# AiRyunn/BoT

Measured on NVIDIA B200. Metric: GAT layer fwd+bwd edges/sec (ogbn-proteins shape), higher is better.
Workload: dtype f32

## Files before the change

bot_b200/_lib.py:

```python
from __future__ import annotations

import ctypes as C
import os

_HERE = os.path.dirname(os.path.abspath(__file__))
LIB_PATH = os.environ.get("BOTGAT_LIB") or os.path.join(_HERE, "libbotgat.so")
ABI_VERSION = 5

c_i64p = C.POINTER(C.c_int64)
c_vp = C.c_void_p

ARRAYS = ("in_indptr", "in_indices", "in_eid", "out_indptr", "out_indices", "out_eid", "in_deg", "out_deg")
ORDER_IN, ORDER_OUT = 0, 1


class GraphInfo(C.Structure):
    _fields_ = [
        ("n_src", C.c_int64), ("n_dst", C.c_int64), ("n_edges", C.c_int64),
        ("max_in_deg", C.c_int64), ("max_out_deg", C.c_int64),
        ("has_zero_in_degree", C.c_int32), ("device", C.c_int32),
        ("n_slots_in", C.c_int64), ("n_slots_out", C.c_int64),
        ("in_eid_identity", C.c_int32), ("tiles_src", C.c_int32), ("tiles_dst", C.c_int32),
        ("n_seg_in", C.c_int32), ("n_seg_out", C.c_int32), ("reserved_", C.c_int32),
    ]


class EdgeSubset(C.Structure):
    _fields_ = [("indptr", c_vp), ("indices", c_vp), ("eid", c_vp), ("kept", c_vp), ("base", c_vp), ("seg_beg", c_vp), ("seg_end", c_vp)]


class FwdArgs(C.Structure):
    _fields_ = [
        ("H", C.c_int32), ("D", C.c_int32),
        ("ld_ft", C.c_int64), ("ld_out", C.c_int64),
        ("ft", c_vp), ("el", c_vp), ("er", c_vp), ("eb", c_vp),
        ("Hb", C.c_int32), ("col_parts", C.c_int32),
        ("am", c_vp), ("ee", c_vp), ("keep", c_vp), ("attn_mul", c_vp), ("src_scale", c_vp), ("dst_scale", c_vp),
        ("slope", C.c_float), ("attn_p", C.c_float), ("seed", C.c_uint64),
        ("out", c_vp), ("row_max", c_vp), ("row_sum", c_vp), ("scratch", c_vp),
        ("h_begin", C.c_int32), ("h_count", C.c_int32),
        ("res", c_vp), ("ld_res", C.c_int64), ("res2", c_vp), ("ld_res2", C.c_int64),
        ("ep_scale", c_vp), ("ep_shift", c_vp), ("y", c_vp), ("ld_y", C.c_int64),
        ("ep_relu", C.c_int32), ("reserved_", C.c_int32),
        ("subset", C.POINTER(EdgeSubset)),
    ]


class BwdArgs(C.Structure):
    _fields_ = [
        ("H", C.c_int32), ("D", C.c_int32),
        ("ld_ft", C.c_int64), ("ld_out", C.c_int64), ("ld_gft", C.c_int64),
        ("ft", c_vp), ("el", c_vp), ("er", c_vp), ("eb_out", c_vp),
        ("Hb", C.c_int32), ("phases", C.c_int32),
        ("am_out", c_vp), ("ee", c_vp), ("keep", c_vp), ("attn_mul", c_vp), ("src_scale", c_vp), ("dst_scale", c_vp),
        ("slope", C.c_float), ("attn_p", C.c_float), ("seed", C.c_uint64),
        ("out", c_vp), ("row_max", c_vp), ("row_sum", c_vp), ("gout", c_vp),
        ("drec", c_vp), ("gprime", c_vp), ("scratch", c_vp), ("gz", c_vp),
        ("grad_ft", c_vp), ("grad_el", c_vp), ("grad_ee", c_vp), ("ld_gee", C.c_int64), ("grad_er", c_vp),
        ("h_begin", C.c_int32), ("h_count", C.c_int32),
        ("subset_out", C.POINTER(EdgeSubset)),
    ]


SIGNATURES = {
    "botgat_abi_version": (C.c_int, []),
# ... 76 lines not shown
```

bot_b200/csrc/common.cuh:

```cuda
#pragma once

#include <atomic>
#include <cuda_runtime.h>
#include <stdint.h>
#include <stdio.h>

#include <type_traits>

#include "botgat.h"

namespace botgat {

void set_error(const char* fmt, ...);
const char* env_str(const char* name);
int64_t env_int(const char* name, int64_t dflt);
extern std::atomic<long long> g_launches;
#define BG_LAUNCHED(n) (::botgat::g_launches.fetch_add(n, std::memory_order_relaxed))

#define BG_CHECK(expr)                                                                  \
  do {                                                                                  \
    cudaError_t _e = (expr);                                                            \
    if (_e != cudaSuccess) {                                                            \
      ::botgat::set_error("%s:%d: %s -> %s", __FILE__, __LINE__, #expr, cudaGetErrorString(_e)); \
      return -2;                                                                        \
    }                                                                                   \
  } while (0)

#define BG_REQUIRE(cond, ...)            \
  do {                                   \
    if (!(cond)) {                       \
      ::botgat::set_error(__VA_ARGS__);  \
      return -1;                         \
    }                                    \
  } while (0)

struct DeviceGuard {
  int prev = -1;
  explicit DeviceGuard(int dev) {
    cudaGetDevice(&prev);
    if (dev != prev) cudaSetDevice(dev);
  }
  ~DeviceGuard() {
    int cur;
    cudaGetDevice(&cur);
    if (cur != prev && prev >= 0) cudaSetDevice(prev);
  }
};

template <typename K>
static inline int resident_grid(K kernel, int block_threads, int64_t blocks_of_work) {
  int dev = 0, sms = 148, per_sm = 1;
  cudaGetDevice(&dev);
  cudaDeviceGetAttribute(&sms, cudaDevAttrMultiProcessorCount, dev);
  if (cudaOccupancyMaxActiveBlocksPerMultiprocessor(&per_sm, kernel, block_threads, 0) != cudaSuccess || per_sm < 1) per_sm = 1;
  const int64_t resident = (int64_t)sms * per_sm;
  return (int)(blocks_of_work < 1 ? 1 : (blocks_of_work < resident ? blocks_of_work : resident));
}

}

struct botgat_graph {
  int device = 0;
  int sm_count = 148;
  int64_t n_src = 0, n_dst = 0, n_edges = 0;
  int64_t max_in_deg = 0, max_out_deg = 0;
  int has_zero_in_degree = 0;
  int32_t *in_indptr = nullptr, *in_indices = nullptr, *in_eid = nullptr;
  int32_t *out_indptr = nullptr, *out_indices = nullptr, *out_eid = nullptr;
  int32_t *in_deg = nullptr, *out_deg = nullptr;
  int in_eid_identity = 0;
  int32_t* out_tile_order = nullptr;
  int tiles_s = 1, tiles_d = 1;
  struct SegTable {
    int n_items = 0;
    int n_slots = 0;
    int n_split = 0;
    int32_t *row = nullptr, *beg = nullptr, *end = nullptr, *slot = nullptr;
    int32_t *split_rows = nullptr, *split_first = nullptr;
  } seg_in, seg_out;
};

namespace botgat {

#ifndef BG_WPB
#define BG_WPB 4
#endif
constexpr int kWarpsPerBlock = BG_WPB;
constexpr unsigned kFull = 0xffffffffu;

__device__ __forceinline__ float leaky_relu(float z, float slope) {
  return z > 0.f ? z : (z == -INFINITY ? -INFINITY : z * slope);
}

__device__ __forceinline__ float warp_max(float v) {
#pragma unroll
  for (int o = 16; o > 0; o >>= 1) v = fmaxf(v, __shfl_xor_sync(kFull, v, o));
  return v;
}
__device__ __forceinline__ float warp_sum(float v) {
#pragma unroll
  for (int o = 16; o > 0; o >>= 1) v += __shfl_xor_sync(kFull, v, o);
  return v;
}

__device__ __forceinline__ uint32_t philox_u32(uint64_t seed, uint32_t eid, uint32_t head) {
  uint32_t c0 = eid, c1 = head >> 2, c2 = 0x9E3779B9u, c3 = 0xBB67AE85u;
  uint32_t k0 = (uint32_t)seed, k1 = (uint32_t)(seed >> 32);
#pragma unroll
  for (int r = 0; r < 10; ++r) {
    uint32_t hi0 = __umulhi(0xD2511F53u, c0), lo0 = 0xD2511F53u * c0;
    uint32_t hi1 = __umulhi(0xCD9E8D57u, c2), lo1 = 0xCD9E8D57u * c2;
    uint32_t n0 = hi1 ^ c1 ^ k0, n1 = lo1, n2 = hi0 ^ c3 ^ k1, n3 = lo0;
    c0 = n0; c1 = n1; c2 = n2; c3 = n3;
    k0 += 0x9E3779B9u; k1 += 0xBB67AE85u;
  }
  uint32_t sel = head & 3u;
  return sel == 0 ? c0 : sel == 1 ? c1 : sel == 2 ? c2 : c3;
}
__device__ __forceinline__ float philox_dropout_mul(uint64_t seed, uint32_t eid, uint32_t head, float p, float inv_keep) {
  float u = (float)(philox_u32(seed, eid, head) >> 8) * (1.0f / 16777216.0f);
  return u >= p ? inv_keep : 0.f;
}

template <int VW> struct Vec;
// ... 119 lines not shown
```

bot_b200/csrc/edge_ops.cu:

```cuda
#include <cub/cub.cuh>
#include <thrust/iterator/counting_iterator.h>
#include <thrust/iterator/transform_iterator.h>

#include "common.cuh"

namespace botgat {

static int env_pf() {
  return (int)env_int("BOTGAT_PF", 0);
}

template <int PF> __device__ __forceinline__ float4 ld_rec4(const float* p) {
  float4 r;
  if constexpr (PF == 64)
    asm("ld.global.nc.L2::64B.v4.f32 {%0,%1,%2,%3}, [%4];" : "=f"(r.x), "=f"(r.y), "=f"(r.z), "=f"(r.w) : "l"(p));
  else if constexpr (PF == 128)
    asm("ld.global.nc.L2::128B.v4.f32 {%0,%1,%2,%3}, [%4];" : "=f"(r.x), "=f"(r.y), "=f"(r.z), "=f"(r.w) : "l"(p));
  else if constexpr (PF == 256)
    asm("ld.global.nc.L2::256B.v4.f32 {%0,%1,%2,%3}, [%4];" : "=f"(r.x), "=f"(r.y), "=f"(r.z), "=f"(r.w) : "l"(p));
  else
    r = __ldg(reinterpret_cast<const float4*>(p));
  return r;
}
template <int PF> __device__ __forceinline__ float2 ld_rec2(const float* p) {
// ... 9 lines not shown
  if constexpr (PF == 64) asm("ld.global.nc.L2::64B.f32 %0, [%1];" : "=f"(r) : "l"(p));
  else if constexpr (PF == 128) asm("ld.global.nc.L2::128B.f32 %0, [%1];" : "=f"(r) : "l"(p));
  else if constexpr (PF == 256) asm("ld.global.nc.L2::256B.f32 %0, [%1];" : "=f"(r) : "l"(p));
  else r = __ldg(p);
  return r;
}

constexpr int kHMax = 8;

template <int VEC, int PF> __device__ __forceinline__ void load_record(const float* rec, int H, float (&v)[kHMax]) {
  if constexpr (VEC == 4) {
#pragma unroll
    for (int q = 0; q < kHMax / 4; ++q) {
      if (q * 4 < H) {
        const float4 t = ld_rec4<PF>(rec + q * 4);
        v[q * 4] = t.x; v[q * 4 + 1] = t.y; v[q * 4 + 2] = t.z; v[q * 4 + 3] = t.w;
      }
    }
  } else if constexpr (VEC == 2) {
#pragma unroll
    for (int q = 0; q < kHMax / 2; ++q) {
      if (q * 2 < H) {
        const float2 t = ld_rec2<PF>(rec + q * 2);
        v[q * 2] = t.x; v[q * 2 + 1] = t.y;
      }
    }
  } else {
#pragma unroll
    for (int q = 0; q < kHMax; ++q)
      if (q < H) v[q] = ld_rec1<PF>(rec + q);
  }
}
template <int VEC> __device__ __forceinline__ void store_record(float* rec, int H, const float (&v)[kHMax]) {
  if constexpr (VEC == 4) {
#pragma unroll
    for (int q = 0; q < kHMax / 4; ++q)
      if (q * 4 < H) *reinterpret_cast<float4*>(rec + q * 4) = make_float4(v[q * 4], v[q * 4 + 1], v[q * 4 + 2], v[q * 4 + 3]);
  } else if constexpr (VEC == 2) {
#pragma unroll
    for (int q = 0; q < kHMax / 2; ++q)
      if (q * 2 < H) *reinterpret_cast<float2*>(rec + q * 2) = make_float2(v[q * 2], v[q * 2 + 1]);
  } else {
#pragma unroll
    for (int q = 0; q < kHMax; ++q)
      if (q < H) rec[q] = v[q];
  }
}

static int record_vec(const void* p, int64_t ld, int H) {
  auto fits = [&](int w) { return ld % w == 0 && ((uintptr_t)p % (4 * w)) == 0 && ((H + w - 1) / w) * w <= ld; };
  return fits(4) ? 4 : (fits(2) ? 2 : 1);
}

__global__ void k_pack_keep(int64_t n_edges, const uint8_t* __restrict__ keep, uint32_t* __restrict__ bits) {
  const int64_t n_round = (n_edges + 31) & ~(int64_t)31;
  for (int64_t e = blockIdx.x * (int64_t)blockDim.x + threadIdx.x; e < n_round; e += (int64_t)gridDim.x * blockDim.x) {
    const unsigned b = __ballot_sync(0xffffffffu, e < n_edges && __ldg(keep + e) != 0);
    if ((threadIdx.x & 31) == 0) bits[e >> 5] = b;
  }
}

struct KeptMap {
  const uint32_t* bits;
  const int32_t* base;
  __device__ __forceinline__ int64_t rank(int64_t x) const {
    return __ldg(base + (x >> 5)) + __popc(__ldg(bits + (x >> 5)) & ((1u << (x & 31)) - 1u));
  }
  __device__ __forceinline__ bool kept(int64_t p) const { return (__ldg(bits + (p >> 5)) >> (p & 31)) & 1u; }
};

template <int VEC, int PF>
__global__ void k_edge_stage(int64_t n_edges, int h0, int Hn, const int32_t* __restrict__ eid,
                             const int32_t* __restrict__ order,
                             const float* __restrict__ src, int64_t ld, const uint8_t* __restrict__ keep,
                             const uint32_t* __restrict__ keep_bits, float* __restrict__ dst,
                             const KeptMap km, const int32_t* __restrict__ indices,
                             int32_t* __restrict__ sub_indices, int32_t* __restrict__ sub_eid) {
  for (int64_t t = blockIdx.x * (int64_t)blockDim.x + threadIdx.x; t < n_edges; t += (int64_t)gridDim.x * blockDim.x) {
    const int64_t p = order ? __ldg(order + t) : t;
    int64_t q = p;
    if (km.bits) {
      if (!km.kept(p)) continue;
      q = km.rank(p);
    }
    const int64_t e = __ldg(eid + p);
    float v[kHMax];
#pragma unroll
    for (int c = 0; c < kHMax; ++c) v[c] = 0.f;
    if (src) load_record<VEC, PF>(src + e * ld + h0, Hn, v);
    const bool dropped = keep_bits ? !((__ldg(keep_bits + (e >> 5)) >> (e & 31)) & 1u) : (keep && !__ldg(keep + e));
#pragma unroll
    for (int c = 0; c < kHMax; ++c)
      if (c < Hn) dst[(int64_t)(h0 + c) * n_edges + q] = dropped ? -INFINITY : v[c];
    if (sub_indices) {
      sub_indices[q] = __ldg(indices + p);
      if (sub_eid) sub_eid[q] = (int32_t)e;
    }
  }
}

template <int VEC>
__global__ void k_edge_unstage(int64_t n_edges, int h0, int Hn, int Hw, const int32_t* __restrict__ eid,
                               const int32_t* __restrict__ order, const KeptMap km,
                               const float* __restrict__ gz, float* __restrict__ dst, int64_t ld) {
  for (int64_t t = blockIdx.x * (int64_t)blockDim.x + threadIdx.x; t < n_edges; t += (int64_t)gridDim.x * blockDim.x) {
    const int64_t p = order ? __ldg(order + t) : t;
    const int64_t e = __ldg(eid + p);
    int64_t q = p;
    bool kept = true;
    if (km.bits) {
      kept = km.kept(p);
      q = km.rank(p);
    }
    float v[kHMax];
#pragma unroll
    for (int c = 0; c < kHMax; ++c) v[c] = (c < Hn && kept) ? __ldg(gz + (int64_t)(h0 + c) * n_edges + q) : 0.f;
    store_record<VEC>(dst + e * ld + h0, Hw, v);
  }
}

__global__ void k_kept_bits(int64_t n_edges, int64_t n_words, const int32_t* __restrict__ eid, const uint8_t* __restrict__ keep,
                            const uint32_t* __restrict__ keep_bits, uint32_t* __restrict__ bits) {
  for (int64_t p = blockIdx.x * (int64_t)blockDim.x + threadIdx.x; p < n_words * 32; p += (int64_t)gridDim.x * blockDim.x) {
    bool k = false;
    if (p < n_edges) {
      const int64_t e = eid ? __ldg(eid + p) : p;
      k = keep_bits ? ((__ldg(keep_bits + (e >> 5)) >> (e & 31)) & 1u) : __ldg(keep + e) != 0;
    }
    const unsigned b = __ballot_sync(0xffffffffu, k);
    if ((threadIdx.x & 31) == 0) bits[p >> 5] = b;
  }
}

struct WordCount {
  const uint32_t* bits;
  __device__ int operator()(int64_t w) const { return __popc(__ldg(bits + w)); }
};

__global__ void k_subset_bounds(int n_rows, const int32_t* __restrict__ indptr, int n_seg, const int32_t* __restrict__ seg_beg,
                                const int32_t* __restrict__ seg_end, const KeptMap km,
                                int32_t* __restrict__ sub_indptr, int32_t* __restrict__ sub_beg, int32_t* __restrict__ sub_end) {
  const int n = max(n_rows + 1, n_seg);
  for (int i = blockIdx.x * blockDim.x + threadIdx.x; i < n; i += gridDim.x * blockDim.x) {
    if (i <= n_rows) sub_indptr[i] = (int32_t)km.rank(__ldg(indptr + i));
    if (i < n_seg) {
      sub_beg[i] = (int32_t)km.rank(__ldg(seg_beg + i));
      sub_end[i] = (int32_t)km.rank(__ldg(seg_end + i));
    }
  }
}

template <int VEC, int PF>
__global__ void __launch_bounds__(256)
k_edge_reduce_dst(int n_items, int H, int h0, int Hn, const int32_t* __restrict__ indptr, const int32_t* __restrict__ eid,
                  const int32_t* __restrict__ seg_row, const int32_t* __restrict__ seg_beg,
                  const int32_t* __restrict__ seg_end, const int32_t* __restrict__ seg_slot,
                  const float* __restrict__ grad_ee, int64_t ld, float* __restrict__ grad_er, float* __restrict__ scratch) {
  const int warp = threadIdx.x >> 5, lane = threadIdx.x & 31;
  const int item = blockIdx.x * 8 + warp;
  if (item >= n_items) return;
  const int v = seg_row ? seg_row[item] : item;
  const int beg = seg_row ? seg_beg[item] : indptr[v], end = seg_row ? seg_end[item] : indptr[v + 1];
  const int slot = seg_row ? seg_slot[item] : -1;
  float s[kHMax];
#pragma unroll
  for (int q = 0; q < kHMax; ++q) s[q] = 0.f;
  for (int pos = beg + lane; pos < end; pos += 32) {
    float r[kHMax];
#pragma unroll
    for (int q = 0; q < kHMax; ++q) r[q] = 0.f;
    load_record<VEC, PF>(grad_ee + (int64_t)__ldg(eid + pos) * ld + h0, Hn, r);
#pragma unroll
    for (int q = 0; q < kHMax; ++q) s[q] += r[q];
  }
#pragma unroll
  for (int q = 0; q < kHMax; ++q) {
    if (q < Hn) {
      const float t = warp_sum(s[q]);
      if (lane == 0) {
        if (slot >= 0) scratch[(int64_t)slot * H + h0 + q] = t;
        else grad_er[(int64_t)v * H + h0 + q] = t;
      }
    }
  }
}

__global__ void k_edge_reduce_combine(int n_split, int H, const int32_t* __restrict__ split_rows,
                                      const int32_t* __restrict__ split_first, const float* __restrict__ scratch,
                                      float* __restrict__ grad_er) {
  const int t = blockIdx.x * blockDim.x + threadIdx.x;
  if (t >= n_split * H) return;
  const int i = t / H, h = t - i * H;
  float a = 0.f;
  for (int s = split_first[i]; s < split_first[i + 1]; ++s) a += scratch[(int64_t)s * H + h];
  grad_er[(int64_t)split_rows[i] * H + h] = a;
}

static inline int grid_for(int64_t n, int block = 256) {
  int64_t b = (n + block - 1) / block;
  return (int)std::max<int64_t>(1, std::min<int64_t>(b, 148 * 32));
}

#define BG_PF_SWITCH(CALL)                        \
  switch (pf) {                                   \
    case 64: { constexpr int PF = 64; CALL; break; }   \
    case 128: { constexpr int PF = 128; CALL; break; } \
    case 256: { constexpr int PF = 256; CALL; break; } \
    default: { constexpr int PF = 0; CALL; break; }    \
  }

struct KeepBits {
  uint32_t* p = nullptr;
  cudaStream_t st = nullptr;
  ~KeepBits() { if (p) cudaFreeAsync(p, st); }
};
static int pack_keep_bits(const botgat_graph* g, const int32_t* eid, const uint8_t* keep, bool with_records, cudaStream_t st,
                          KeepBits* kb) {
  const bool coalesced = eid == g->in_eid && g->in_eid_identity;
  if (!keep || !with_records || g->n_edges < (1 << 20) || coalesced) return 0;
  kb->st = st;
  BG_CHECK(cudaMallocAsync(&kb->p, sizeof(uint32_t) * (size_t)((g->n_edges + 31) / 32), st));
  k_pack_keep<<<grid_for(g->n_edges), 256, 0, st>>>(g->n_edges, keep, kb->p);
  BG_LAUNCHED(1);
  return 0;
}

static int build_subset(const botgat_graph* g, int order, const uint8_t* keep, const uint32_t* keep_bits,
                        botgat_edge_subset* s, cudaStream_t st) {
  const bool in = order == BOTGAT_ORDER_IN;
  const int32_t* eid = in ? g->in_eid : g->out_eid;
  const botgat_graph::SegTable& seg = in ? g->seg_in : g->seg_out;
  const int n_rows = (int)(in ? g->n_dst : g->n_src);
  const int n_seg = seg.n_items;
  const int64_t n_words = g->n_edges / 32 + 1;
  k_kept_bits<<<grid_for(n_words * 32), 256, 0, st>>>(g->n_edges, n_words, in && g->in_eid_identity ? nullptr : eid, keep,
                                                      keep_bits, s->kept);
  BG_LAUNCHED(1);
  auto counts = thrust::make_transform_iterator(thrust::counting_iterator<int64_t>(0), WordCount{s->kept});
  size_t tb = 0;
  BG_CHECK(cub::DeviceScan::ExclusiveSum(nullptr, tb, counts, s->base, (int)n_words, st));
  void* tmp = nullptr;
  BG_CHECK(cudaMallocAsync(&tmp, tb, st));
  const cudaError_t scan = cub::DeviceScan::ExclusiveSum(tmp, tb, counts, s->base, (int)n_words, st);
  BG_LAUNCHED(1);
  BG_CHECK(cudaFreeAsync(tmp, st));
  BG_CHECK(scan);
  const KeptMap km{s->kept, s->base};
  k_subset_bounds<<<grid_for(std::max(n_rows + 1, n_seg)), 256, 0, st>>>(n_rows, in ? g->in_indptr : g->out_indptr, n_seg,
                                                                        seg.beg, seg.end, km, s->indptr, s->seg_beg,
                                                                        s->seg_end);
  BG_LAUNCHED(1);
  BG_CHECK(cudaGetLastError());
  return 0;
}

static int stage_one(const botgat_graph* g, const int32_t* eid, const int32_t* order, int H, const float* src, int64_t ld,
                     const uint8_t* keep, float* dst, const botgat_edge_subset* sub, const int32_t* indices,
                     cudaStream_t st) {
  const int pf = env_pf();
  KeepBits kb;
  if (int rc = pack_keep_bits(g, eid, keep, src != nullptr, st, &kb)) return rc;
  const uint32_t* keep_bits = kb.p;
  const KeptMap km{sub ? sub->kept : nullptr, sub ? sub->base : nullptr};
  for (int h0 = 0; h0 < H; h0 += kHMax) {
    const int Hn = std::min(kHMax, H - h0);
    const int vec = src ? record_vec(src + h0, ld, Hn) : 1;
    int32_t* sub_indices = sub && indices && h0 == 0 ? sub->indices : nullptr;
    int32_t* sub_eid = sub_indices ? sub->eid : nullptr;
    const int grid = order ? (int)((g->n_edges + 255) / 256) : grid_for(g->n_edges);
#define BG_ST(VEC) BG_PF_SWITCH((k_edge_stage<VEC, PF><<<grid, 256, 0, st>>>(g->n_edges, h0, Hn, eid, order, src, ld, keep, keep_bits, dst, km, indices, sub_indices, sub_eid)))
    if (vec == 4) { BG_ST(4) } else if (vec == 2) { BG_ST(2) } else { BG_ST(1) }
#undef BG_ST
    BG_LAUNCHED(1);
    BG_CHECK(cudaGetLastError());
  }
  return 0;
}

}

using namespace botgat;

extern "C" int botgat_edge_stage(const botgat_graph* g, int order, int32_t H, const float* ee, int64_t ld_ee,
                                 const uint8_t* keep, const float* attn_mul, int64_t ld_am, float* eb, float* am,
                                 botgat_edge_subset* subset, void* stream) {
  BG_REQUIRE(g && H > 0, "edge_stage: bad arguments");
  BG_REQUIRE(order == BOTGAT_ORDER_IN || order == BOTGAT_ORDER_OUT, "edge_stage: bad order %d", order);
  BG_REQUIRE((eb != nullptr) == (ee != nullptr || keep != nullptr), "edge_stage: eb must be given iff ee or keep is");
  BG_REQUIRE((am != nullptr) == (attn_mul != nullptr), "edge_stage: am must be given iff attn_mul is");
  BG_REQUIRE(!ee || ld_ee >= H, "edge_stage: ld_ee < H");
  BG_REQUIRE(!attn_mul || ld_am >= H, "edge_stage: ld_am < H");
  BG_REQUIRE(!subset || keep, "edge_stage: the kept-edge subset needs keep");
  const bool split = (order == BOTGAT_ORDER_IN ? g->seg_in : g->seg_out).n_items > 0;
  BG_REQUIRE(!subset || (subset->kept && subset->base && subset->indptr && subset->indices &&
                         (!split || (subset->seg_beg && subset->seg_end))),
             "edge_stage: subset needs kept, base, indptr, indices and, for a CSR with split rows, seg_beg / seg_end");
  DeviceGuard guard(g->device);
  cudaStream_t st = (cudaStream_t)stream;
  if (g->n_edges == 0) {
    if (subset)
      BG_CHECK(cudaMemsetAsync(subset->indptr, 0, sizeof(int32_t) * (size_t)((order == BOTGAT_ORDER_IN ? g->n_dst : g->n_src) + 1), st));
    return 0;
  }
  if (!eb && !am) return 0;
  const int32_t* eid = order == BOTGAT_ORDER_IN ? g->in_eid : g->out_eid;
  const int32_t* visit = order == BOTGAT_ORDER_OUT ? g->out_tile_order : nullptr;
  if (subset) {
    KeepBits kb;
    int rc = pack_keep_bits(g, eid, keep, ee != nullptr, st, &kb);
    if (!rc) rc = build_subset(g, order, keep, kb.p, subset, st);
    if (rc) return rc;
  }
  const int32_t* indices = order == BOTGAT_ORDER_IN ? g->in_indices : g->out_indices;
  if (eb) {
    int rc = stage_one(g, eid, visit, ee ? H : 1, ee, ld_ee, subset ? nullptr : keep, eb, subset, indices, st);
    if (rc) return rc;
  }
  if (am) {
    int rc = stage_one(g, eid, visit, H, attn_mul, ld_am, nullptr, am, subset, nullptr, st);
    if (rc) return rc;
  }
  return 0;
}

extern "C" int botgat_edge_unstage(const botgat_graph* g, int order, int32_t H, const float* gz, float* grad_ee,
                                   int64_t ld_gee, const botgat_edge_subset* subset, void* stream) {
  BG_REQUIRE(g && H > 0, "edge_unstage: bad arguments");
  BG_REQUIRE(order == BOTGAT_ORDER_IN || order == BOTGAT_ORDER_OUT, "edge_unstage: bad order %d", order);
  if (g->n_edges == 0) return 0;
  BG_REQUIRE(gz && grad_ee, "edge_unstage: null gz/grad_ee");
  BG_REQUIRE(ld_gee >= H, "edge_unstage: ld_gee < H");
  BG_REQUIRE(!subset || (subset->kept && subset->base), "edge_unstage: subset without kept / base");
  DeviceGuard guard(g->device);
  cudaStream_t st = (cudaStream_t)stream;
  const int32_t* eid = order == BOTGAT_ORDER_IN ? g->in_eid : g->out_eid;
  const int32_t* visit = order == BOTGAT_ORDER_OUT ? g->out_tile_order : nullptr;
  const KeptMap km{subset ? subset->kept : nullptr, subset ? subset->base : nullptr};
  for (int h0 = 0; h0 < ld_gee; h0 += kHMax) {
    const int Hn = std::max(0, std::min(kHMax, H - h0));
    const int Hw = (int)std::min<int64_t>(kHMax, ld_gee - h0);
    const int vec = record_vec(grad_ee + h0, ld_gee, Hw);
    const int grid = visit ? (int)((g->n_edges + 255) / 256) : grid_for(g->n_edges);
    if (vec == 4) k_edge_unstage<4><<<grid, 256, 0, st>>>(g->n_edges, h0, Hn, Hw, eid, visit, km, gz, grad_ee, ld_gee);
    else if (vec == 2) k_edge_unstage<2><<<grid, 256, 0, st>>>(g->n_edges, h0, Hn, Hw, eid, visit, km, gz, grad_ee, ld_gee);
    else k_edge_unstage<1><<<grid, 256, 0, st>>>(g->n_edges, h0, Hn, Hw, eid, visit, km, gz, grad_ee, ld_gee);
    BG_LAUNCHED(1);
    BG_CHECK(cudaGetLastError());
  }
  return 0;
}

extern "C" int botgat_edge_reduce_dst(const botgat_graph* g, int32_t H, const float* grad_ee, int64_t ld_gee,
                                      float* grad_er, float* scratch, void* stream) {
  BG_REQUIRE(g && H > 0 && grad_er, "edge_reduce_dst: bad arguments");
  BG_REQUIRE(grad_ee || g->n_edges == 0, "edge_reduce_dst: null grad_ee");
  BG_REQUIRE(ld_gee >= H || g->n_edges == 0, "edge_reduce_dst: ld_gee < H");
  if (g->n_dst == 0) return 0;
  DeviceGuard guard(g->device);
  cudaStream_t st = (cudaStream_t)stream;
  const int pf = env_pf();
  const botgat_graph::SegTable& seg = g->seg_in;
  const bool split = seg.n_items > 0;
  BG_REQUIRE(!split || seg.n_slots == 0 || scratch, "edge_reduce_dst: this graph has split rows; scratch (n_slots_in*H floats) is required");
  const int n_items = split ? seg.n_items : (int)g->n_dst;
  const int32_t *sr = split ? seg.row : nullptr, *sb = seg.beg, *se = seg.end, *ss = seg.slot;
  const int grid = (n_items + 7) / 8;
  for (int h0 = 0; h0 < H; h0 += kHMax) {
    const int Hn = std::min(kHMax, H - h0);
    const int vec = g->n_edges ? record_vec(grad_ee + h0, ld_gee, Hn) : 1;
#define BG_RD(VEC) BG_PF_SWITCH((k_edge_reduce_dst<VEC, PF><<<grid, 256, 0, st>>>(n_items, H, h0, Hn, g->in_indptr, g->in_eid, sr, sb, se, ss, grad_ee, ld_gee, grad_er, scratch)))
    if (vec == 4) { BG_RD(4) } else if (vec == 2) { BG_RD(2) } else { BG_RD(1) }
#undef BG_RD
    BG_LAUNCHED(1);
    BG_CHECK(cudaGetLastError());
  }
  if (split && seg.n_split > 0) {
    const int n = seg.n_split * H;
    k_edge_reduce_combine<<<(n + 255) / 256, 256, 0, st>>>(seg.n_split, H, seg.split_rows, seg.split_first, scratch, grad_er);
    BG_LAUNCHED(1);
    BG_CHECK(cudaGetLastError());
  }
  return 0;
}
```

bot_b200/csrc/graph.cu:

```cuda
#include <cub/cub.cuh>

#include <atomic>
#include <cstdarg>
#include <cstring>

#include "common.cuh"

namespace botgat {

static thread_local char g_err[512] = "";
std::atomic<long long> g_launches{0};

void set_error(const char* fmt, ...) {
  va_list ap;
  va_start(ap, fmt);
  vsnprintf(g_err, sizeof(g_err), fmt, ap);
  va_end(ap);
}

__global__ void k_narrow_and_check(int64_t n, const int64_t* __restrict__ a, int64_t bound, int32_t* __restrict__ out,
                                   int32_t* __restrict__ iota, int* __restrict__ bad) {
  for (int64_t i = blockIdx.x * (int64_t)blockDim.x + threadIdx.x; i < n; i += (int64_t)gridDim.x * blockDim.x) {
    const int64_t v = a[i];
    const bool oob = v < 0 || v >= bound;
// ... 71 lines not shown
    void* tmp = nullptr;
    BG_CHECK(cudaMallocAsync(&tmp, tmp_bytes, st));
    BG_CHECK(cub::DeviceRadixSort::SortPairs(tmp, tmp_bytes, key, key_sorted_tmp, iota, eid, (int)n_edges, 0,
                                             bits_for(n_rows), st)); BG_LAUNCHED(1);
    BG_CHECK(cudaFreeAsync(tmp, st));
    k_gather_i32<<<grid_for(n_edges), 256, 0, st>>>(n_edges, other, eid, indices); BG_LAUNCHED(1);
    BG_CHECK(cudaGetLastError());
  }
  BG_CHECK(cudaMemsetAsync(deg, 0, sizeof(int32_t) * (n_rows + 1), st));
  if (n_edges > 0) {
    k_histogram<<<grid_for(n_edges), 256, 0, st>>>(n_edges, key, deg); BG_LAUNCHED(1);
    BG_CHECK(cudaGetLastError());
  }
  {
    size_t tmp_bytes = 0;
    BG_CHECK(cub::DeviceScan::ExclusiveSum(nullptr, tmp_bytes, deg, indptr, (int)(n_rows + 1), st));
    void* tmp = nullptr;
    BG_CHECK(cudaMallocAsync(&tmp, tmp_bytes, st));
    BG_CHECK(cub::DeviceScan::ExclusiveSum(tmp, tmp_bytes, deg, indptr, (int)(n_rows + 1), st)); BG_LAUNCHED(1);
    BG_CHECK(cudaFreeAsync(tmp, st));
  }
  return 0;
}

}

using namespace botgat;

extern "C" int botgat_abi_version(void) { return BOTGAT_ABI_VERSION; }
extern "C" const char* botgat_last_error(void) { return g_err; }
extern "C" int64_t botgat_launch_count(void) { return (int64_t)g_launches.load(); }

static void configure_pool(int device) {
  static std::atomic<unsigned> done{0};
  const unsigned bit = 1u << (device & 31);
  if (done.fetch_or(bit) & bit) return;
  cudaMemPool_t pool;
  if (cudaDeviceGetDefaultMemPool(&pool, device) != cudaSuccess) return;
  uint64_t thr = 0;
  if (cudaMemPoolGetAttribute(pool, cudaMemPoolAttrReleaseThreshold, &thr) == cudaSuccess && thr == 0) {
    thr = 2ull << 30;
    cudaMemPoolSetAttribute(pool, cudaMemPoolAttrReleaseThreshold, &thr);
  }
}

static void destroy_impl(botgat_graph* g, bool async, cudaStream_t st) {
  if (!g) return;
  DeviceGuard guard(g->device);
  void* ptrs[] = {g->in_indptr, g->in_indices, g->in_eid, g->out_indptr, g->out_indices, g->out_eid, g->in_deg, g->out_deg};
  for (void* q : ptrs) {
    if (!q) continue;
    if (!async || cudaFreeAsync(q, st) != cudaSuccess) { cudaGetLastError(); cudaFree(q); }
  }
  if (g->out_tile_order && (!async || cudaFreeAsync(g->out_tile_order, st) != cudaSuccess)) { cudaGetLastError(); cudaFree(g->out_tile_order); }
  free_segments(&g->seg_in, async, st); free_segments(&g->seg_out, async, st);
  delete g;
}

extern "C" void botgat_graph_destroy(botgat_graph* g) { destroy_impl(g, false, nullptr); }
extern "C" void botgat_graph_destroy_async(botgat_graph* g, void* stream) { destroy_impl(g, true, (cudaStream_t)stream); }

extern "C" int botgat_graph_create(int64_t n_src, int64_t n_dst, int64_t n_edges, const int64_t* src,
                                   const int64_t* dst, int device, void* stream, botgat_graph** out) {
  BG_REQUIRE(out, "graph_create: null out");
  *out = nullptr;
  BG_REQUIRE(n_src >= 0 && n_dst >= 0 && n_edges >= 0, "graph_create: negative size");
  BG_REQUIRE(n_edges < (1ll << 31) - 1 && n_src < (1ll << 31) - 1 && n_dst < (1ll << 31) - 1,
             "graph_create: sizes must be < 2^31-1 (int32 structure arrays)");
  BG_REQUIRE(n_edges == 0 || (src && dst), "graph_create: null src/dst");
  DeviceGuard guard(device);
  cudaStream_t st = (cudaStream_t)stream;

  botgat_graph* g = new botgat_graph();
  g->device = device; g->n_src = n_src; g->n_dst = n_dst; g->n_edges = n_edges;
  cudaDeviceGetAttribute(&g->sm_count, cudaDevAttrMultiProcessorCount, device);
  struct Cleanup {
    botgat_graph*& g;
    bool armed = true;
    ~Cleanup() { if (armed) { botgat_graph_destroy(g); } }
  } cleanup{g};

  configure_pool(device);
  const size_t eb = sizeof(int32_t) * (size_t)std::max<int64_t>(n_edges, 1);
  BG_CHECK(cudaMallocAsync(&g->in_indptr, sizeof(int32_t) * (n_dst + 1), st));
  BG_CHECK(cudaMallocAsync(&g->out_indptr, sizeof(int32_t) * (n_src + 1), st));
  BG_CHECK(cudaMallocAsync(&g->in_indices, eb, st)); BG_CHECK(cudaMallocAsync(&g->in_eid, eb, st));
  BG_CHECK(cudaMallocAsync(&g->out_indices, eb, st)); BG_CHECK(cudaMallocAsync(&g->out_eid, eb, st));
  BG_CHECK(cudaMallocAsync(&g->in_deg, sizeof(int32_t) * (n_dst + 1), st));
  BG_CHECK(cudaMallocAsync(&g->out_deg, sizeof(int32_t) * (n_src + 1), st));

  int32_t *src32 = nullptr, *dst32 = nullptr, *iota = nullptr, *ktmp = nullptr;
  int* flags = nullptr;
  BG_CHECK(cudaMallocAsync(&src32, eb, st)); BG_CHECK(cudaMallocAsync(&dst32, eb, st));
  BG_CHECK(cudaMallocAsync(&iota, eb, st)); BG_CHECK(cudaMallocAsync(&ktmp, eb, st));
  BG_CHECK(cudaMallocAsync(&flags, sizeof(int) * 6, st));
  BG_CHECK(cudaMemsetAsync(flags, 0, sizeof(int) * 6, st));
  if (n_edges > 0) {
    k_narrow_and_check<<<grid_for(n_edges), 256, 0, st>>>(n_edges, src, n_src, src32, iota, flags); BG_LAUNCHED(1);
    k_narrow_and_check<<<grid_for(n_edges), 256, 0, st>>>(n_edges, dst, n_dst, dst32, nullptr, flags); BG_LAUNCHED(1);
    BG_CHECK(cudaGetLastError());
  }
  int rc = build_csr(n_dst, n_edges, dst32, src32, iota, ktmp, g->in_indptr, g->in_indices, g->in_eid, g->in_deg, st);
  if (rc) return rc;
  rc = build_csr(n_src, n_edges, src32, dst32, iota, ktmp, g->out_indptr, g->out_indices, g->out_eid, g->out_deg, st);
  if (rc) return rc;
  if (n_dst > 0) k_deg_stats<<<grid_for(n_dst), 256, 0, st>>>(n_dst, g->in_deg, flags + 1); BG_LAUNCHED(1);
  if (n_src > 0) k_deg_stats<<<grid_for(n_src), 256, 0, st>>>(n_src, g->out_deg, flags + 3); BG_LAUNCHED(1);
  if (n_edges > 0) k_check_identity<<<grid_for(n_edges), 256, 0, st>>>(n_edges, g->in_eid, flags + 5); BG_LAUNCHED(1);
  BG_CHECK(cudaGetLastError());
  int h[6];
  BG_CHECK(cudaMemcpyAsync(h, flags, sizeof(h), cudaMemcpyDeviceToHost, st));
  BG_CHECK(cudaFreeAsync(src32, st)); BG_CHECK(cudaFreeAsync(dst32, st));
  BG_CHECK(cudaFreeAsync(flags, st));
  BG_CHECK(cudaStreamSynchronize(st));
  if (h[0] != 0) { cudaFreeAsync(iota, st); cudaFreeAsync(ktmp, st); }
  BG_REQUIRE(h[0] == 0, "graph_create: node id out of range [0,n_src) / [0,n_dst)");
  g->max_in_deg = h[1]; g->has_zero_in_degree = h[2] > 0; g->max_out_deg = h[3];
  g->in_eid_identity = h[5] == 0;
  {
    int ts = 1, td = 1;
    const char* force = env_str("BOTGAT_TILES");
    if (force) {
      if (sscanf(force, "%d,%d", &ts, &td) != 2) ts = td = 1;
    } else if (g->in_eid_identity && n_edges >= (1 << 22) && n_src > 0 && n_dst > 0) {
      const double avg_in = (double)n_edges / n_dst, avg_out = (double)n_edges / n_src;
      const int cap_s = std::max(1, (int)(avg_in / 16)), cap_d = std::max(1, (int)(avg_out / 16));
      const double need = (double)n_edges * 32.0 / ((double)env_int("BOTGAT_TILE_MB", 20) * (1 << 20));
      int want = 1;
      while ((double)want * want < need) ++want;
      ts = std::min(want, cap_s); td = std::min(want, cap_d);
      while ((double)ts * td < need && ts < cap_s) ++ts;
      while ((double)ts * td < need && td < cap_d) ++td;
      if ((double)ts * td < need * 0.5) ts = td = 1;
    }
    ts = std::max(1, std::min(ts, 64)); td = std::max(1, std::min(td, 64));
    if (ts * td > 1 && n_edges > 0 && n_src > 0 && n_dst > 0) {
      const int rows_per_s = (int)((n_src + ts - 1) / ts), rows_per_d = (int)((n_dst + td - 1) / td);
      BG_CHECK(cudaMallocAsync(&g->out_tile_order, eb, st));
      k_tile_keys<<<grid_for(n_src * 32), 256, 0, st>>>((int)n_src, g->out_indptr, g->out_indices, rows_per_s, rows_per_d,
                                                       td, ktmp, iota); BG_LAUNCHED(1);
      int32_t* ksorted = nullptr;
      BG_CHECK(cudaMallocAsync(&ksorted, eb, st));
      size_t tmp_bytes = 0;
      const int kbits = bits_for((int64_t)ts * td);
      BG_CHECK(cub::DeviceRadixSort::SortPairs(nullptr, tmp_bytes, ktmp, ksorted, iota, g->out_tile_order, (int)n_edges, 0, kbits, st));
      void* tmp = nullptr;
      BG_CHECK(cudaMallocAsync(&tmp, tmp_bytes, st));
      BG_CHECK(cub::DeviceRadixSort::SortPairs(tmp, tmp_bytes, ktmp, ksorted, iota, g->out_tile_order, (int)n_edges, 0, kbits, st)); BG_LAUNCHED(1);
      BG_CHECK(cudaFreeAsync(tmp, st)); BG_CHECK(cudaFreeAsync(ksorted, st));
      g->tiles_s = ts; g->tiles_d = td;
    }
  }
  BG_CHECK(cudaFreeAsync(iota, st)); BG_CHECK(cudaFreeAsync(ktmp, st));
  rc = build_segments((int)n_dst, g->in_indptr, g->in_deg, g->max_in_deg, &g->seg_in, st);
  if (rc) return rc;
  rc = build_segments((int)n_src, g->out_indptr, g->out_deg, g->max_out_deg, &g->seg_out, st);
  if (rc) return rc;
  cleanup.armed = false;
  *out = g;
  return 0;
}

extern "C" int botgat_graph_get(const botgat_graph* g, int which, void** dev_ptr, int64_t* len) {
  BG_REQUIRE(g && dev_ptr && len, "graph_get: null argument");
  switch (which) {
    case BOTGAT_IN_INDPTR: *dev_ptr = g->in_indptr; *len = g->n_dst + 1; break;
    case BOTGAT_IN_INDICES: *dev_ptr = g->in_indices; *len = g->n_edges; break;
    case BOTGAT_IN_EID: *dev_ptr = g->in_eid; *len = g->n_edges; break;
    case BOTGAT_OUT_INDPTR: *dev_ptr = g->out_indptr; *len = g->n_src + 1; break;
    case BOTGAT_OUT_INDICES: *dev_ptr = g->out_indices; *len = g->n_edges; break;
    case BOTGAT_OUT_EID: *dev_ptr = g->out_eid; *len = g->n_edges; break;
    case BOTGAT_IN_DEG: *dev_ptr = g->in_deg; *len = g->n_dst; break;
    case BOTGAT_OUT_DEG: *dev_ptr = g->out_deg; *len = g->n_src; break;
    default: set_error("graph_get: unknown array %d", which); return -1;
  }
  return 0;
}

extern "C" int botgat_graph_get_info(const botgat_graph* g, botgat_graph_info* info) {
  BG_REQUIRE(g && info, "graph_get_info: null argument");
  info->n_src = g->n_src; info->n_dst = g->n_dst; info->n_edges = g->n_edges;
  info->max_in_deg = g->max_in_deg; info->max_out_deg = g->max_out_deg;
  info->has_zero_in_degree = g->has_zero_in_degree; info->device = g->device;
  info->n_slots_in = g->seg_in.n_slots; info->n_slots_out = g->seg_out.n_slots;
  info->in_eid_identity = g->in_eid_identity; info->tiles_src = g->tiles_s; info->tiles_dst = g->tiles_d;
  info->n_seg_in = g->seg_in.n_items; info->n_seg_out = g->seg_out.n_items; info->reserved_ = 0;
  return 0;
}

namespace botgat {

__global__ void k_pack_bidirected(int64_t n, const int64_t* __restrict__ src, const int64_t* __restrict__ dst,
                                  int64_t n_nodes, uint64_t* __restrict__ keys, int* __restrict__ bad) {
  for (int64_t i = blockIdx.x * (int64_t)blockDim.x + threadIdx.x; i < n; i += (int64_t)gridDim.x * blockDim.x) {
    const int64_t s = src[i], d = dst[i];
    if (s < 0 || s >= n_nodes || d < 0 || d >= n_nodes) *bad = 1;
    keys[i] = (uint64_t)s * (uint64_t)n_nodes + (uint64_t)d;
    keys[n + i] = (uint64_t)d * (uint64_t)n_nodes + (uint64_t)s;
  }
}
__global__ void k_unpack(int64_t n, const uint64_t* __restrict__ keys, int64_t n_nodes, int64_t* __restrict__ src,
                         int64_t* __restrict__ dst) {
  for (int64_t i = blockIdx.x * (int64_t)blockDim.x + threadIdx.x; i < n; i += (int64_t)gridDim.x * blockDim.x) {
    src[i] = (int64_t)(keys[i] / (uint64_t)n_nodes);
    dst[i] = (int64_t)(keys[i] % (uint64_t)n_nodes);
  }
}
__global__ void k_flag_not_loop(int64_t n, const int64_t* __restrict__ src, const int64_t* __restrict__ dst,
                                uint8_t* __restrict__ flag) {
  for (int64_t i = blockIdx.x * (int64_t)blockDim.x + threadIdx.x; i < n; i += (int64_t)gridDim.x * blockDim.x)
    flag[i] = src[i] != dst[i];
}
__global__ void k_iota64(int64_t n, int64_t* __restrict__ a, int64_t* __restrict__ b) {
  for (int64_t i = blockIdx.x * (int64_t)blockDim.x + threadIdx.x; i < n; i += (int64_t)gridDim.x * blockDim.x) {
    a[i] = i;
    b[i] = i;
  }
}

}

extern "C" int botgat_coo_to_bidirected(int64_t n_nodes, int64_t n_edges, const int64_t* src, const int64_t* dst,
                                        int64_t* out_src, int64_t* out_dst, int64_t* n_out, int device, void* stream) {
  BG_REQUIRE(n_out, "to_bidirected: null n_out");
  *n_out = 0;
  if (n_edges == 0) return 0;
// ... 222 lines not shown
```

include/botgat.h:

```cpp
#ifndef BOTGAT_H_
#define BOTGAT_H_

#include <stdint.h>

#ifdef __cplusplus
extern "C" {
#endif
#if defined(__GNUC__)
#pragma GCC visibility push(default)
#endif

#define BOTGAT_ABI_VERSION 5

typedef struct botgat_graph botgat_graph;

int botgat_abi_version(void);
const char* botgat_last_error(void);
int64_t botgat_launch_count(void);

int botgat_graph_create(int64_t n_src, int64_t n_dst, int64_t n_edges,
                        const int64_t* src, const int64_t* dst,
                        int device, void* stream, botgat_graph** out);
void botgat_graph_destroy(botgat_graph* g);
void botgat_graph_destroy_async(botgat_graph* g, void* stream);

enum {
  BOTGAT_IN_INDPTR = 0,
  BOTGAT_IN_INDICES = 1,
  BOTGAT_IN_EID = 2,
  BOTGAT_OUT_INDPTR = 3,
  BOTGAT_OUT_INDICES = 4,
  BOTGAT_OUT_EID = 5,
  BOTGAT_IN_DEG = 6,
  BOTGAT_OUT_DEG = 7
};
int botgat_graph_get(const botgat_graph* g, int which, void** dev_ptr, int64_t* len);

typedef struct {
  int64_t n_src, n_dst, n_edges;
  int64_t max_in_deg, max_out_deg;
  int32_t has_zero_in_degree;
  int32_t device;
  int64_t n_slots_in, n_slots_out;
  int32_t in_eid_identity;
  int32_t tiles_src, tiles_dst;
  int32_t n_seg_in, n_seg_out;
  int32_t reserved_;
} botgat_graph_info;
int botgat_graph_get_info(const botgat_graph* g, botgat_graph_info* info );

int botgat_coo_to_bidirected(int64_t n_nodes, int64_t n_edges,
                             const int64_t* src, const int64_t* dst,
                             int64_t* out_src, int64_t* out_dst, int64_t* n_out,
                             int device, void* stream);
int botgat_coo_remove_self_loop(int64_t n_edges, const int64_t* src, const int64_t* dst,
                                int64_t* out_src, int64_t* out_dst, int64_t* n_out,
                                int device, void* stream);
int botgat_coo_add_self_loop(int64_t n_nodes, int64_t n_edges,
                             const int64_t* src, const int64_t* dst,
                             int64_t* out_src, int64_t* out_dst,
                             int device, void* stream);

enum { BOTGAT_ORDER_IN = 0, BOTGAT_ORDER_OUT = 1 };
typedef struct {
  int32_t* indptr;
  int32_t* indices;
  int32_t* eid;
  uint32_t* kept;
  int32_t* base;
  int32_t* seg_beg;
  int32_t* seg_end;
} botgat_edge_subset;
int botgat_edge_stage(const botgat_graph* g, int order, int32_t H,
                      const float* ee, int64_t ld_ee, const uint8_t* keep,
                      const float* attn_mul, int64_t ld_am,
                      float* eb, float* am, botgat_edge_subset* subset , void* stream);
int botgat_edge_unstage(const botgat_graph* g, int order, int32_t H, const float* gz,
                        float* grad_ee, int64_t ld_gee, const botgat_edge_subset* subset ,
                        void* stream);
int botgat_edge_reduce_dst(const botgat_graph* g, int32_t H, const float* grad_ee, int64_t ld_gee,
                           float* grad_er, float* scratch ,
                           void* stream);

int botgat_edge_proj_gw_blocks(void);
int botgat_edge_proj_forward(int64_t n, int32_t C, int32_t H, const float* x, int64_t ld_x, const float* W,
                             float* y, int64_t ld_y, int device, void* stream);
int botgat_edge_proj_backward(int64_t n, int32_t C, int32_t H, const float* x, int64_t ld_x, const float* W,
// ... 125 lines not shown
```

Before: 2.896 billion.

## Precompute tile-ordered eid/indices and batch two edges per thread in stage kernels

At graph build time, the out-edge eid and neighbor index arrays are gathered into tile visit order, so the stage and unstage kernels read them contiguously instead of through a second dependent indirection. The stage and unstage kernels now process two positions per thread and issue all loads before any stores to raise memory-level parallelism. The in-order eid lookup is skipped when in_eid is the identity. The keep-bit packing is routed through an existing kernel. This costs two extra int32 edge arrays in memory and adds register pressure.

```diff
diff --git a/bot_b200/_lib.py b/bot_b200/_lib.py
--- a/bot_b200/_lib.py
+++ b/bot_b200/_lib.py
@@ -10,7 +10,8 @@
 c_i64p = C.POINTER(C.c_int64)
 c_vp = C.c_void_p
 
-ARRAYS = ("in_indptr", "in_indices", "in_eid", "out_indptr", "out_indices", "out_eid", "in_deg", "out_deg")
+ARRAYS = ("in_indptr", "in_indices", "in_eid", "out_indptr", "out_indices", "out_eid", "in_deg", "out_deg",
+          "out_tile_order", "out_tile_eid", "out_tile_indices")
 ORDER_IN, ORDER_OUT = 0, 1
 
 
diff --git a/bot_b200/csrc/common.cuh b/bot_b200/csrc/common.cuh
--- a/bot_b200/csrc/common.cuh
+++ b/bot_b200/csrc/common.cuh
@@ -70,6 +70,7 @@
   int32_t *in_deg = nullptr, *out_deg = nullptr;
   int in_eid_identity = 0;
   int32_t* out_tile_order = nullptr;
+  int32_t *out_tile_eid = nullptr, *out_tile_indices = nullptr;
   int tiles_s = 1, tiles_d = 1;
   struct SegTable {
     int n_items = 0;
diff --git a/bot_b200/csrc/edge_ops.cu b/bot_b200/csrc/edge_ops.cu
--- a/bot_b200/csrc/edge_ops.cu
+++ b/bot_b200/csrc/edge_ops.cu
@@ -85,70 +85,101 @@
   return fits(4) ? 4 : (fits(2) ? 2 : 1);
 }
 
-__global__ void k_pack_keep(int64_t n_edges, const uint8_t* __restrict__ keep, uint32_t* __restrict__ bits) {
-  const int64_t n_round = (n_edges + 31) & ~(int64_t)31;
-  for (int64_t e = blockIdx.x * (int64_t)blockDim.x + threadIdx.x; e < n_round; e += (int64_t)gridDim.x * blockDim.x) {
-    const unsigned b = __ballot_sync(0xffffffffu, e < n_edges && __ldg(keep + e) != 0);
-    if ((threadIdx.x & 31) == 0) bits[e >> 5] = b;
-  }
-}
-
 struct KeptMap {
   const uint32_t* bits;
   const int32_t* base;
   __device__ __forceinline__ int64_t rank(int64_t x) const {
     return __ldg(base + (x >> 5)) + __popc(__ldg(bits + (x >> 5)) & ((1u << (x & 31)) - 1u));
   }
-  __device__ __forceinline__ bool kept(int64_t p) const { return (__ldg(bits + (p >> 5)) >> (p & 31)) & 1u; }
 };
 
+constexpr int kPos = 2;
 template <int VEC, int PF>
-__global__ void k_edge_stage(int64_t n_edges, int h0, int Hn, const int32_t* __restrict__ eid,
-                             const int32_t* __restrict__ order,
-                             const float* __restrict__ src, int64_t ld, const uint8_t* __restrict__ keep,
-                             const uint32_t* __restrict__ keep_bits, float* __restrict__ dst,
-                             const KeptMap km, const int32_t* __restrict__ indices,
-                             int32_t* __restrict__ sub_indices, int32_t* __restrict__ sub_eid) {
-  for (int64_t t = blockIdx.x * (int64_t)blockDim.x + threadIdx.x; t < n_edges; t += (int64_t)gridDim.x * blockDim.x) {
-    const int64_t p = order ? __ldg(order + t) : t;
-    int64_t q = p;
-    if (km.bits) {
-      if (!km.kept(p)) continue;
-      q = km.rank(p);
-    }
-    const int64_t e = __ldg(eid + p);
-    float v[kHMax];
-#pragma unroll
-    for (int c = 0; c < kHMax; ++c) v[c] = 0.f;
-    if (src) load_record<VEC, PF>(src + e * ld + h0, Hn, v);
-    const bool dropped = keep_bits ? !((__ldg(keep_bits + (e >> 5)) >> (e & 31)) & 1u) : (keep && !__ldg(keep + e));
-#pragma unroll
-    for (int c = 0; c < kHMax; ++c)
-      if (c < Hn) dst[(int64_t)(h0 + c) * n_edges + q] = dropped ? -INFINITY : v[c];
-    if (sub_indices) {
-      sub_indices[q] = __ldg(indices + p);
-      if (sub_eid) sub_eid[q] = (int32_t)e;
+__global__ void __launch_bounds__(256)
+k_edge_stage(int64_t n_edges, int h0, int Hn, const int32_t* __restrict__ eid, const int32_t* __restrict__ order,
+             const int32_t* __restrict__ teid, const int32_t* __restrict__ tidx,
+             const float* __restrict__ src, int64_t ld, const uint8_t* __restrict__ keep,
+             const uint32_t* __restrict__ keep_bits, float* __restrict__ dst,
+             const KeptMap km, const int32_t* __restrict__ indices,
+             int32_t* __restrict__ sub_indices, int32_t* __restrict__ sub_eid) {
+  const int64_t step = (int64_t)gridDim.x * blockDim.x * kPos;
+  for (int64_t t0 = blockIdx.x * (int64_t)blockDim.x * kPos + threadIdx.x; t0 < n_edges; t0 += step) {
+    int64_t p[kPos], e[kPos];
+    int32_t nb[kPos];
+#pragma unroll
+    for (int k = 0; k < kPos; ++k) {
+      const int64_t t = min(t0 + (int64_t)k * blockDim.x, n_edges - 1);
+      p[k] = order ? __ldg(order + t) : t;
+      e[k] = teid ? __ldg(teid + t) : (eid ? __ldg(eid + p[k]) : p[k]);
+      nb[k] = sub_indices ? (tidx ? __ldg(tidx + t) : __ldg(indices + p[k])) : 0;
+    }
+    float v[kPos][kHMax];
+    bool dropped[kPos];
+    uint32_t kw[kPos];
+    int32_t kb[kPos];
+#pragma unroll
+    for (int k = 0; k < kPos; ++k) {
+#pragma unroll
+      for (int c = 0; c < kHMax; ++c) v[k][c] = 0.f;
+      if (src) load_record<VEC, PF>(src + e[k] * ld + h0, Hn, v[k]);
+      dropped[k] = keep_bits ? !((__ldg(keep_bits + (e[k] >> 5)) >> (e[k] & 31)) & 1u) : (keep && !__ldg(keep + e[k]));
+      kw[k] = km.bits ? __ldg(km.bits + (p[k] >> 5)) : 0u;
+      kb[k] = km.bits ? __ldg(km.base + (p[k] >> 5)) : 0;
+    }
+#pragma unroll
+    for (int k = 0; k < kPos; ++k) {
+      if (t0 + (int64_t)k * blockDim.x >= n_edges) break;
+      int64_t q = p[k];
+      if (km.bits) {
+        const uint32_t below = (1u << (p[k] & 31)) - 1u;
+        if (!((kw[k] >> (p[k] & 31)) & 1u)) continue;
+        q = kb[k] + __popc(kw[k] & below);
+      }
+#pragma unroll
+      for (int c = 0; c < kHMax; ++c)
+        if (c < Hn) dst[(int64_t)(h0 + c) * n_edges + q] = dropped[k] ? -INFINITY : v[k][c];
+      if (sub_indices) {
+        sub_indices[q] = nb[k];
+        if (sub_eid) sub_eid[q] = (int32_t)e[k];
+      }
     }
   }
 }
 
 template <int VEC>
-__global__ void k_edge_unstage(int64_t n_edges, int h0, int Hn, int Hw, const int32_t* __restrict__ eid,
-                               const int32_t* __restrict__ order, const KeptMap km,
-                               const float* __restrict__ gz, float* __restrict__ dst, int64_t ld) {
-  for (int64_t t = blockIdx.x * (int64_t)blockDim.x + threadIdx.x; t < n_edges; t += (int64_t)gridDim.x * blockDim.x) {
-    const int64_t p = order ? __ldg(order + t) : t;
-    const int64_t e = __ldg(eid + p);
-    int64_t q = p;
-    bool kept = true;
-    if (km.bits) {
-      kept = km.kept(p);
-      q = km.rank(p);
-    }
-    float v[kHMax];
-#pragma unroll
-    for (int c = 0; c < kHMax; ++c) v[c] = (c < Hn && kept) ? __ldg(gz + (int64_t)(h0 + c) * n_edges + q) : 0.f;
-    store_record<VEC>(dst + e * ld + h0, Hw, v);
+__global__ void __launch_bounds__(256)
+k_edge_unstage(int64_t n_edges, int h0, int Hn, int Hw, const int32_t* __restrict__ eid,
+               const int32_t* __restrict__ order, const int32_t* __restrict__ teid, const KeptMap km,
+               const float* __restrict__ gz, float* __restrict__ dst, int64_t ld) {
+  const int64_t step = (int64_t)gridDim.x * blockDim.x * kPos;
+  for (int64_t t0 = blockIdx.x * (int64_t)blockDim.x * kPos + threadIdx.x; t0 < n_edges; t0 += step) {
+    int64_t p[kPos], e[kPos];
+#pragma unroll
+    for (int k = 0; k < kPos; ++k) {
+      const int64_t t = min(t0 + (int64_t)k * blockDim.x, n_edges - 1);
+      p[k] = order ? __ldg(order + t) : t;
+      e[k] = teid ? __ldg(teid + t) : (eid ? __ldg(eid + p[k]) : p[k]);
+    }
+    int64_t q[kPos];
+    bool kept[kPos];
+#pragma unroll
+    for (int k = 0; k < kPos; ++k) {
+      q[k] = p[k];
+      kept[k] = true;
+      if (km.bits) {
+        const uint32_t w = __ldg(km.bits + (p[k] >> 5));
+        kept[k] = (w >> (p[k] & 31)) & 1u;
+        q[k] = __ldg(km.base + (p[k] >> 5)) + __popc(w & ((1u << (p[k] & 31)) - 1u));
+      }
+    }
+    float v[kPos][kHMax];
+#pragma unroll
+    for (int k = 0; k < kPos; ++k)
+#pragma unroll
+      for (int c = 0; c < kHMax; ++c) v[k][c] = (c < Hn && kept[k]) ? __ldg(gz + (int64_t)(h0 + c) * n_edges + q[k]) : 0.f;
+#pragma unroll
+    for (int k = 0; k < kPos; ++k)
+      if (t0 + (int64_t)k * blockDim.x < n_edges) store_record<VEC>(dst + e[k] * ld + h0, Hw, v[k]);
   }
 }
 
@@ -202,7 +233,7 @@
     float r[kHMax];
 #pragma unroll
     for (int q = 0; q < kHMax; ++q) r[q] = 0.f;
-    load_record<VEC, PF>(grad_ee + (int64_t)__ldg(eid + pos) * ld + h0, Hn, r);
+    load_record<VEC, PF>(grad_ee + (eid ? (int64_t)__ldg(eid + pos) : (int64_t)pos) * ld + h0, Hn, r);
 #pragma unroll
     for (int q = 0; q < kHMax; ++q) s[q] += r[q];
   }
@@ -253,7 +284,8 @@
   if (!keep || !with_records || g->n_edges < (1 << 20) || coalesced) return 0;
   kb->st = st;
   BG_CHECK(cudaMallocAsync(&kb->p, sizeof(uint32_t) * (size_t)((g->n_edges + 31) / 32), st));
-  k_pack_keep<<<grid_for(g->n_edges), 256, 0, st>>>(g->n_edges, keep, kb->p);
+  const int64_t n_words = (g->n_edges + 31) / 32;
+  k_kept_bits<<<grid_for(n_words * 32), 256, 0, st>>>(g->n_edges, n_words, nullptr, keep, nullptr, kb->p);
   BG_LAUNCHED(1);
   return 0;
 }
@@ -287,7 +319,20 @@
   return 0;
 }
 
-static int stage_one(const botgat_graph* g, const int32_t* eid, const int32_t* order, int H, const float* src, int64_t ld,
+struct Walk {
+  const int32_t *eid, *order, *teid, *tidx;
+};
+static Walk walk_of(const botgat_graph* g, int order) {
+  if (order == BOTGAT_ORDER_IN) return {g->in_eid_identity ? nullptr : g->in_eid, nullptr, nullptr, nullptr};
+  return {g->out_eid, g->out_tile_order, g->out_tile_eid, g->out_tile_indices};
+}
+
+static int walk_grid(const botgat_graph* g, const Walk& w) {
+  const int64_t per_block = 256 * (int64_t)kPos;
+  return w.order ? (int)((g->n_edges + per_block - 1) / per_block) : grid_for((g->n_edges + kPos - 1) / kPos);
+}
+
+static int stage_one(const botgat_graph* g, const int32_t* eid, const Walk& w, int H, const float* src, int64_t ld,
                      const uint8_t* keep, float* dst, const botgat_edge_subset* sub, const int32_t* indices,
                      cudaStream_t st) {
   const int pf = env_pf();
@@ -295,13 +340,13 @@
   if (int rc = pack_keep_bits(g, eid, keep, src != nullptr, st, &kb)) return rc;
   const uint32_t* keep_bits = kb.p;
   const KeptMap km{sub ? sub->kept : nullptr, sub ? sub->base : nullptr};
+  const int grid = walk_grid(g, w);
   for (int h0 = 0; h0 < H; h0 += kHMax) {
     const int Hn = std::min(kHMax, H - h0);
     const int vec = src ? record_vec(src + h0, ld, Hn) : 1;
     int32_t* sub_indices = sub && indices && h0 == 0 ? sub->indices : nullptr;
     int32_t* sub_eid = sub_indices ? sub->eid : nullptr;
-    const int grid = order ? (int)((g->n_edges + 255) / 256) : grid_for(g->n_edges);
-#define BG_ST(VEC) BG_PF_SWITCH((k_edge_stage<VEC, PF><<<grid, 256, 0, st>>>(g->n_edges, h0, Hn, eid, order, src, ld, keep, keep_bits, dst, km, indices, sub_indices, sub_eid)))
+#define BG_ST(VEC) BG_PF_SWITCH((k_edge_stage<VEC, PF><<<grid, 256, 0, st>>>(g->n_edges, h0, Hn, w.eid, w.order, w.teid, w.tidx, src, ld, keep, keep_bits, dst, km, indices, sub_indices, sub_eid)))
     if (vec == 4) { BG_ST(4) } else if (vec == 2) { BG_ST(2) } else { BG_ST(1) }
 #undef BG_ST
     BG_LAUNCHED(1);
@@ -337,7 +382,7 @@
   }
   if (!eb && !am) return 0;
   const int32_t* eid = order == BOTGAT_ORDER_IN ? g->in_eid : g->out_eid;
-  const int32_t* visit = order == BOTGAT_ORDER_OUT ? g->out_tile_order : nullptr;
+  const Walk w = walk_of(g, order);
   if (subset) {
     KeepBits kb;
     int rc = pack_keep_bits(g, eid, keep, ee != nullptr, st, &kb);
@@ -346,11 +391,11 @@
   }
   const int32_t* indices = order == BOTGAT_ORDER_IN ? g->in_indices : g->out_indices;
   if (eb) {
-    int rc = stage_one(g, eid, visit, ee ? H : 1, ee, ld_ee, subset ? nullptr : keep, eb, subset, indices, st);
+    int rc = stage_one(g, eid, w, ee ? H : 1, ee, ld_ee, subset ? nullptr : keep, eb, subset, indices, st);
     if (rc) return rc;
   }
   if (am) {
-    int rc = stage_one(g, eid, visit, H, attn_mul, ld_am, nullptr, am, subset, nullptr, st);
+    int rc = stage_one(g, eid, w, H, attn_mul, ld_am, nullptr, am, subset, nullptr, st);
     if (rc) return rc;
   }
   return 0;
@@ -366,17 +411,16 @@
   BG_REQUIRE(!subset || (subset->kept && subset->base), "edge_unstage: subset without kept / base");
   DeviceGuard guard(g->device);
   cudaStream_t st = (cudaStream_t)stream;
-  const int32_t* eid = order == BOTGAT_ORDER_IN ? g->in_eid : g->out_eid;
-  const int32_t* visit = order == BOTGAT_ORDER_OUT ? g->out_tile_order : nullptr;
+  const Walk w = walk_of(g, order);
   const KeptMap km{subset ? subset->kept : nullptr, subset ? subset->base : nullptr};
+  const int grid = walk_grid(g, w);
   for (int h0 = 0; h0 < ld_gee; h0 += kHMax) {
     const int Hn = std::max(0, std::min(kHMax, H - h0));
     const int Hw = (int)std::min<int64_t>(kHMax, ld_gee - h0);
     const int vec = record_vec(grad_ee + h0, ld_gee, Hw);
-    const int grid = visit ? (int)((g->n_edges + 255) / 256) : grid_for(g->n_edges);
-    if (vec == 4) k_edge_unstage<4><<<grid, 256, 0, st>>>(g->n_edges, h0, Hn, Hw, eid, visit, km, gz, grad_ee, ld_gee);
-    else if (vec == 2) k_edge_unstage<2><<<grid, 256, 0, st>>>(g->n_edges, h0, Hn, Hw, eid, visit, km, gz, grad_ee, ld_gee);
-    else k_edge_unstage<1><<<grid, 256, 0, st>>>(g->n_edges, h0, Hn, Hw, eid, visit, km, gz, grad_ee, ld_gee);
+#define BG_UN(VEC) k_edge_unstage<VEC><<<grid, 256, 0, st>>>(g->n_edges, h0, Hn, Hw, w.eid, w.order, w.teid, km, gz, grad_ee, ld_gee);
+    if (vec == 4) { BG_UN(4) } else if (vec == 2) { BG_UN(2) } else { BG_UN(1) }
+#undef BG_UN
     BG_LAUNCHED(1);
     BG_CHECK(cudaGetLastError());
   }
@@ -401,7 +445,7 @@
   for (int h0 = 0; h0 < H; h0 += kHMax) {
     const int Hn = std::min(kHMax, H - h0);
     const int vec = g->n_edges ? record_vec(grad_ee + h0, ld_gee, Hn) : 1;
-#define BG_RD(VEC) BG_PF_SWITCH((k_edge_reduce_dst<VEC, PF><<<grid, 256, 0, st>>>(n_items, H, h0, Hn, g->in_indptr, g->in_eid, sr, sb, se, ss, grad_ee, ld_gee, grad_er, scratch)))
+#define BG_RD(VEC) BG_PF_SWITCH((k_edge_reduce_dst<VEC, PF><<<grid, 256, 0, st>>>(n_items, H, h0, Hn, g->in_indptr, g->in_eid_identity ? nullptr : g->in_eid, sr, sb, se, ss, grad_ee, ld_gee, grad_er, scratch)))
     if (vec == 4) { BG_RD(4) } else if (vec == 2) { BG_RD(2) } else { BG_RD(1) }
 #undef BG_RD
     BG_LAUNCHED(1);
diff --git a/bot_b200/csrc/graph.cu b/bot_b200/csrc/graph.cu
--- a/bot_b200/csrc/graph.cu
+++ b/bot_b200/csrc/graph.cu
@@ -147,7 +147,8 @@
     if (!q) continue;
     if (!async || cudaFreeAsync(q, st) != cudaSuccess) { cudaGetLastError(); cudaFree(q); }
   }
-  if (g->out_tile_order && (!async || cudaFreeAsync(g->out_tile_order, st) != cudaSuccess)) { cudaGetLastError(); cudaFree(g->out_tile_order); }
+  for (void* q : {(void*)g->out_tile_order, (void*)g->out_tile_eid, (void*)g->out_tile_indices})
+    if (q && (!async || cudaFreeAsync(q, st) != cudaSuccess)) { cudaGetLastError(); cudaFree(q); }
   free_segments(&g->seg_in, async, st); free_segments(&g->seg_out, async, st);
   delete g;
 }
@@ -243,6 +244,10 @@
       BG_CHECK(cudaMallocAsync(&tmp, tmp_bytes, st));
       BG_CHECK(cub::DeviceRadixSort::SortPairs(tmp, tmp_bytes, ktmp, ksorted, iota, g->out_tile_order, (int)n_edges, 0, kbits, st)); BG_LAUNCHED(1);
       BG_CHECK(cudaFreeAsync(tmp, st)); BG_CHECK(cudaFreeAsync(ksorted, st));
+      BG_CHECK(cudaMallocAsync(&g->out_tile_eid, eb, st)); BG_CHECK(cudaMallocAsync(&g->out_tile_indices, eb, st));
+      k_gather_i32<<<grid_for(n_edges), 256, 0, st>>>(n_edges, g->out_eid, g->out_tile_order, g->out_tile_eid); BG_LAUNCHED(1);
+      k_gather_i32<<<grid_for(n_edges), 256, 0, st>>>(n_edges, g->out_indices, g->out_tile_order, g->out_tile_indices); BG_LAUNCHED(1);
+      BG_CHECK(cudaGetLastError());
       g->tiles_s = ts; g->tiles_d = td;
     }
   }
@@ -267,6 +272,9 @@
     case BOTGAT_OUT_EID: *dev_ptr = g->out_eid; *len = g->n_edges; break;
     case BOTGAT_IN_DEG: *dev_ptr = g->in_deg; *len = g->n_dst; break;
     case BOTGAT_OUT_DEG: *dev_ptr = g->out_deg; *len = g->n_src; break;
+    case BOTGAT_OUT_TILE_ORDER: *dev_ptr = g->out_tile_order; *len = g->out_tile_order ? g->n_edges : 0; break;
+    case BOTGAT_OUT_TILE_EID: *dev_ptr = g->out_tile_eid; *len = g->out_tile_eid ? g->n_edges : 0; break;
+    case BOTGAT_OUT_TILE_INDICES: *dev_ptr = g->out_tile_indices; *len = g->out_tile_indices ? g->n_edges : 0; break;
     default: set_error("graph_get: unknown array %d", which); return -1;
   }
   return 0;
diff --git a/include/botgat.h b/include/botgat.h
--- a/include/botgat.h
+++ b/include/botgat.h
@@ -32,7 +32,10 @@
   BOTGAT_OUT_INDICES = 4,
   BOTGAT_OUT_EID = 5,
   BOTGAT_IN_DEG = 6,
-  BOTGAT_OUT_DEG = 7
+  BOTGAT_OUT_DEG = 7,
+  BOTGAT_OUT_TILE_ORDER = 8,
+  BOTGAT_OUT_TILE_EID = 9,
+  BOTGAT_OUT_TILE_INDICES = 10
 };
 int botgat_graph_get(const botgat_graph* g, int which, void** dev_ptr, int64_t* len);
 
```

Result: faster. 2.939 billion (median of 6 runs) (+1.5%).
